# unclearness/vacancy

Hardware: AMD Instinct MI355X
Metric: Mvoxel*views/s (Carve) (higher is better)
Workload: dtype f32

## Files before the change

### vacancy_amd/csrc/carve_fused_device.h

```cpp
#pragma once
#include "carve_fused.h"

namespace vcy {
namespace {

#define VCY_SETPRIO(n) __builtin_amdgcn_s_setprio(n)

#ifdef VCY_PHASE_TIMING
__device__ unsigned long long g_phase_ticks[256][16];
#define VCY_PT_DECL unsigned long long pt_last = __builtin_amdgcn_s_memtime(), pt_acc[16] = {0, 0, 0, 0, 0, 0, 0, 0, 0, 0, 0, 0, 0, 0, 0, 0}
#define VCY_PT(slot)                                                  \
  do {                                                                \
    const unsigned long long t_ = __builtin_amdgcn_s_memtime();       \
    pt_acc[slot] += t_ - pt_last;                                     \
    pt_last = t_;                                                     \
  } while (0)
#define VCY_PT_COUNT(slot) pt_acc[slot] += 1
#define VCY_PT_FLUSH(lane_)                                                                         \
  do {                                                                                              \
    if ((lane_) == 0)                                                                               \
      for (int q_ = 0; q_ < 16; ++q_) atomicAdd(&g_phase_ticks[blockIdx.x & 255][q_], pt_acc[q_]);  \
  } while (0)
#else
#define VCY_PT_DECL
// ... 27 lines not shown
}

__device__ __forceinline__ float div_view1(int div, float n, float d) {
  float r = __builtin_amdgcn_rcpf(d);
  if (div == 1) {
    const float e = __builtin_fmaf(-d, r, 1.0f);
    r = __builtin_fmaf(e, r, r);
  }
  const float q = n * r;
  const float e2 = __builtin_fmaf(-d, q, n);
  return __builtin_fmaf(e2, r, q);
}

__device__ __forceinline__ bool in_fast_div_range(float z) {
  const unsigned lo = 0x21800000u;
  const unsigned hi = 0x5d800000u;
  return (__float_as_uint(z) - lo) <= (hi - lo);
}

typedef const float __attribute__((address_space(1))) * gfloat_ptr;
__device__ __forceinline__ float load_u32_index(gfloat_ptr base, unsigned idx) {
  typedef const char __attribute__((address_space(1))) * gchar_ptr;
  return *(gfloat_ptr)((gchar_ptr)base + (idx << 2));
}
typedef const float __attribute__((address_space(4))) * cfloat_ptr;
__device__ __attribute__((noinline)) bool sample_generic(const ViewParams* v, ModeParams m, float px,
                                                         float py, float pz, float* dist) {
  return view_distance<true, 0, 0, false, false>(*v, m, px, py, pz, dist);
}

__device__ __forceinline__ void wave_lds_fence() {
  __builtin_amdgcn_fence(__ATOMIC_RELEASE, "wavefront");
  __builtin_amdgcn_wave_barrier();
  __builtin_amdgcn_fence(__ATOMIC_ACQUIRE, "wavefront");
}

__device__ __forceinline__ float rcp_count(float m) {
  const float r = __builtin_amdgcn_rcpf(m);
  const float e = __builtin_fmaf(-m, r, 1.0f);
  return __builtin_fmaf(e, r, r);
}

template <int UPDATE>
__device__ __forceinline__ bool apply_sample(bool ok, float dist, float wgt, float& s, int& n) {
  if (UPDATE == VCY_UPDATE_MAX) {
    const bool take = ok && (n < 1 || dist > s);
    s = take ? dist : s;
    n += take ? 1 : 0;
    return take;
  } else if (UPDATE == kUpdateWaUnitWeight) {
    const float inv_denom = rcp_count((float)(n + 1));
    const float avg = ((float)n * s + dist) * inv_denom;
    const float ns = (n < 1) ? dist : avg;
    s = ok ? ns : s;
    n += ok ? 1 : 0;
  } else {
    const float inv_denom = div_fast(1.0f, wgt * (float)(n + 1));
    const float avg = (wgt * (float)n * s + wgt * dist) * inv_denom;
    const float ns = (n < 1) ? dist : avg;
    s = ok ? ns : s;
    n += ok ? 1 : 0;
  }
  return ok;
}

__device__ __forceinline__ void update_max_touched(float dist, float& s, int& n, unsigned long long& took) {
  asm("v_cmp_gt_f32_e32 vcc, %[d], %[s]\n\t"
      "s_or_b64 %[took], %[took], vcc\n\t"
      "v_cndmask_b32_e32 %[s], %[s], %[d], vcc\n\t"
      "v_addc_co_u32_e32 %[n], vcc, 0, %[n], vcc"
      : [s] "+v"(s), [n] "+v"(n), [took] "+s"(took)
      : [d] "v"(dist)
      : "vcc");
}

template <bool TRUNC>
__device__ __forceinline__ void update_wa_unit(float dist, float& s, float& fn, unsigned long long& took) {
  const float f1 = fn + 1.0f;
  const float avg = (fn * s + dist) * rcp_count(f1);
  if (TRUNC) {
    asm("v_cmp_ngt_f32_e32 vcc, -1.0, %[d]\n\t"
        "s_or_b64 %[took], %[took], vcc\n\t"
        "v_cndmask_b32_e32 %[s], %[s], %[avg], vcc\n\t"
        "v_cndmask_b32_e32 %[fn], %[fn], %[f1], vcc"
        : [s] "+v"(s), [fn] "+v"(fn), [took] "+s"(took)
        : [d] "v"(dist), [avg] "v"(avg), [f1] "v"(f1)
        : "vcc");
  } else {
    s = avg;
    fn = f1;
  }
}

typedef float f4 __attribute__((ext_vector_type(4)));
typedef f4 __attribute__((address_space(3))) lds_float4;

template <int UPDATE>
__device__ __forceinline__ bool apply_sample(bool ok, float dist, float wgt, float& s, float& fn) {
  const float f1 = fn + 1.0f;
  float avg;
  if (UPDATE == kUpdateWaUnitWeight) {
    avg = (fn * s + dist) * rcp_count(f1);
  } else {
    avg = (wgt * fn * s + wgt * dist) * div_fast(1.0f, wgt * f1);
  }
  const float ns = (fn < 1.0f) ? dist : avg;
  s = ok ? ns : s;
  fn = ok ? f1 : fn;
  return ok;
}

__device__ __forceinline__ int div_small(int q, float inv) { return (int)(((float)q + 0.5f) * inv); }

typedef float __attribute__((address_space(3))) lds_float;
typedef uint32_t __attribute__((address_space(3))) lds_u32;

__device__ __forceinline__ void raw_prefetch(const ViewParams& v, const TileInfo& ti, int lane, float* buf) {
#ifdef VCY_FLOOR_NO_TILE_LOADS
  return;
#endif
  asm volatile("" : "+v"(lane));
  const int nq = __builtin_amdgcn_readfirstlane(ti.nq);
  if (nq == 0) return;
  const int th = __builtin_amdgcn_readfirstlane(ti.th);
  const int tx0 = __builtin_amdgcn_readfirstlane(ti.tx0);
  const int ty0 = __builtin_amdgcn_readfirstlane(ti.ty0);
  gfloat_ptr img = (gfloat_ptr)v.sdf;
  const unsigned width = (unsigned)v.width;
  lds_float* dst = (lds_float*)buf;
  if (tx0 + 15 <= v.roi_max_xi && ty0 + 15 <= v.roi_max_yi) {
    const unsigned lane_off = __umul24(width, (unsigned)lane >> 4) + ((unsigned)lane & 15u);
    gfloat_ptr base = img + (__umul24(width, (unsigned)ty0) + (unsigned)tx0);
#pragma unroll
    for (int r = 0; r < 4; ++r) {
      if (4 * r <= th)
        __builtin_amdgcn_global_load_lds(base + (size_t)(4 * r) * width + lane_off, dst + 64 * r, 4, 0, 0);
    }
    return;
  }
  const unsigned xx = (unsigned)min(tx0 + (lane & 15), v.roi_max_xi);
  const int yl = ty0 + (lane >> 4);
#pragma unroll
  for (int r = 0; r < 4; ++r) {
    if (4 * r <= th) {
      const unsigned yy = (unsigned)min(yl + 4 * r, v.roi_max_yi);
      __builtin_amdgcn_global_load_lds(img + (__umul24(width, yy) + xx), dst + 64 * r, 4, 0, 0);
    }
  }
}

__device__ __forceinline__ void raw_tile_wait() { asm volatile("s_waitcnt vmcnt(0)" ::: "memory"); }

__device__ __forceinline__ float wave_min(float v) {
#define VCY_DPP_MIN(CTRL) asm volatile("s_nop 1\n\tv_min_f32_dpp %0, %0, %0 " CTRL : "+v"(v))
  VCY_DPP_MIN("quad_perm:[1,0,3,2] row_mask:0xf bank_mask:0xf");
  VCY_DPP_MIN("quad_perm:[2,3,0,1] row_mask:0xf bank_mask:0xf");
  VCY_DPP_MIN("row_half_mirror row_mask:0xf bank_mask:0xf");
  VCY_DPP_MIN("row_mirror row_mask:0xf bank_mask:0xf");
  VCY_DPP_MIN("row_bcast:15 row_mask:0xa bank_mask:0xf");
  VCY_DPP_MIN("row_bcast:31 row_mask:0xc bank_mask:0xf");
#undef VCY_DPP_MIN
  return __uint_as_float(__builtin_amdgcn_readlane(__float_as_uint(v), 63));
}

__device__ __forceinline__ void tile_fill(const ViewParams& v, const TileInfo& ti, int lane, float* tile) {
  const int nq = __builtin_amdgcn_readfirstlane(ti.nq);
  if (nq == 0) return;
  const int tw = __builtin_amdgcn_readfirstlane(ti.tw), th = __builtin_amdgcn_readfirstlane(ti.th);
  const int tx0 = __builtin_amdgcn_readfirstlane(ti.tx0);
  const int ty0 = __builtin_amdgcn_readfirstlane(ti.ty0);
  const float inv_pitch = __uint_as_float(__builtin_amdgcn_readfirstlane(__float_as_uint(ti.inv_tw)));
  const int pitch = tw + 1, npx = pitch * (th + 1);
  gfloat_ptr img = (gfloat_ptr)v.sdf;
  const unsigned width = (unsigned)v.width;
  lds_float* dst = (lds_float*)tile;
  for (int q0 = 0; q0 < npx; q0 += 64) {
    const int q = q0 + lane;
    if (q < npx) {
      const int j = div_small(q, inv_pitch), i = q - j * pitch;
      const unsigned xx = (unsigned)min(tx0 + i, v.roi_max_xi), yy = (unsigned)min(ty0 + j, v.roi_max_yi);
      __builtin_amdgcn_global_load_lds(img + (__umul24(width, yy) + xx), dst + q0, 4, 0, 0);
    }
  }
  raw_tile_wait();
}

template <bool SAMEF, int TQ, bool GEN>
__device__ __forceinline__ TileInfo footprint_of(const FusedView& fv, float xl, float xh, float yl, float yh, float zl_,
                                                 float zh, bool is_ortho, bool outside_max, bool want_bound,
                                                 bool want_lower, float* lower_out = nullptr) {
  const ViewParams& v = fv.v;
  const float xa = fmaxf(fabsf(xl), fabsf(xh)), ya = fmaxf(fabsf(yl), fabsf(yh)), za = fmaxf(fabsf(zl_), fabsf(zh));
  const bool ortho = GEN && is_ortho;
  float p0[3], ax[3], ay[3], az[3], mag[3];
#pragma unroll
  for (int i = 0; i < 3; ++i) {
    p0[i] = v.t[i] + (v.r[i][0] * xl + (v.r[i][1] * yl + v.r[i][2] * zl_));
    ax[i] = v.r[i][0] * (xh - xl);
    ay[i] = v.r[i][1] * (yh - yl);
    az[i] = v.r[i][2] * (zh - zl_);
    mag[i] = fabsf(v.t[i]) + (fabsf(v.r[i][0]) * xa + (fabsf(v.r[i][1]) * ya + fabsf(v.r[i][2]) * za));
  }
  float umin = INFINITY, umax = -INFINITY, wmin = INFINITY, wmax_ = -INFINITY, zmin = INFINITY, zmax = -INFINITY;
  int bad = 0;
  const float fx = v.fx, fy = SAMEF ? v.fx : v.fy;
  float pxy[4][3];
#pragma unroll
  for (int i = 0; i < 3; ++i) {
    pxy[0][i] = p0[i];
    pxy[1][i] = p0[i] + ax[i];
    pxy[2][i] = p0[i] + ay[i];
    pxy[3][i] = pxy[1][i] + ay[i];
  }
#pragma unroll
  for (int corner = 0; corner < 8; ++corner) {
    float pc[3];
#pragma unroll
    for (int i = 0; i < 3; ++i) pc[i] = (corner & 4) ? pxy[corner & 3][i] + az[i] : pxy[corner & 3][i];
    float u = pc[0], w = pc[1];
    if (!ortho) {
      const float rz = __builtin_amdgcn_rcpf(pc[2]);
      u = __builtin_fmaf(fx * rz, pc[0], v.cx);
      w = __builtin_fmaf(fy * rz, pc[1], v.cy);
    }
    umin = fminf(umin, u);
    umax = fmaxf(umax, u);
    wmin = fminf(wmin, w);
    wmax_ = fmaxf(wmax_, w);
    zmin = fminf(zmin, pc[2]);
    zmax = fmaxf(zmax, pc[2]);
  }
  if (!ortho) bad |= !in_fast_div_range(zmin) || !in_fast_div_range(zmax);
  bad |= !(mag[0] < 0x1p60f) || !(mag[1] < 0x1p60f) || !(mag[2] < 0x1p60f);
  bad |= !(umin > -1.0e6f) || !(umax < 1.0e6f) || !(wmin > -1.0e6f) || !(wmax_ < 1.0e6f);
  const float uabs = fmaxf(fabsf(umin), fabsf(umax)), wabs = fmaxf(fabsf(wmin), fabsf(wmax_));
  float err_u, err_w;
  if (ortho) {
    err_u = 0x1p-21f * mag[0];
    err_w = 0x1p-21f * mag[1];
  } else {
    bad |= !(zmin * 4.0f >= zmax);
    const float iz = 0x1p-21f * __builtin_amdgcn_rcpf(zmin) * 1.0001f;
    err_u = iz * (fx * mag[0] + (uabs + fabsf(v.cx)) * mag[2]) + 0x1p-21f * (uabs + fabsf(v.cx));
    err_w = iz * (fy * mag[1] + (wabs + fabsf(v.cy)) * mag[2]) + 0x1p-21f * (wabs + fabsf(v.cy));
  }
  const float margin = 0.125f;
  bad |= !(err_u <= 0.03125f) || !(err_w <= 0.03125f);
  TileInfo ti;
  ti.lo_x = ti.lo_y = INFINITY;
  ti.hi_x = ti.hi_y = -INFINITY;
  ti.pitchf = 0.0f;
  ti.base = 0;
  ti.tx0 = ti.ty0 = ti.tw = ti.nq = ti.th = 0;
  ti.inv_tw = 1.0f;
  ti.ub = INFINITY;
  ti.sure = 0;
  if (!bad) {
    const int tx0 = max((int)floorf(umin - margin), v.roi_min_xi);
    const int ty0 = max((int)floorf(wmin - margin), v.roi_min_yi);
    const int tx1 = min((int)floorf(umax + margin), v.roi_max_xi);
    const int ty1 = min((int)floorf(wmax_ + margin), v.roi_max_yi);
    const int tw = tx1 - tx0 + 1, th = ty1 - ty0 + 1;
    constexpr bool kRaw = TQ == kTileRaw;
    if (tw > 0 && th > 0 && (kRaw ? (tw <= 15 && th <= 15) : ((tw + 1) * (th + 1) <= kBigPixels))) {
      const bool unclipped = (int)floorf(umin - margin) >= v.roi_min_xi && (int)floorf(wmin - margin) >= v.roi_min_yi &&
                             (int)floorf(umax + margin) < v.roi_max_xi && (int)floorf(wmax_ + margin) < v.roi_max_yi;
      const bool depth_ok = 0x1p-20f * mag[2] <= 0.25f * zmin && zmin >= 0x1p-58f && zmax <= 0x1p58f;
      const int pitch = kRaw ? 16 : tw + 1;
      const bool small_base = ty0 * pitch + tx0 < (1 << 18);
      const bool depth_ok_ortho = zmin > 0x1p-20f * mag[2];
      ti.sure = (unclipped && (ortho ? depth_ok_ortho : depth_ok) && small_base) ? 1 : 0;
      ti.tx0 = tx0;
      ti.ty0 = ty0;
      ti.tw = tw;
      ti.th = th;
      ti.nq = tw * th;
      ti.inv_tw = 1.0f / (float)pitch;
      ti.pitchf = (float)pitch;
      ti.base = -(ty0 * pitch + tx0);
      ti.lo_x = (float)tx0;
      ti.lo_y = (float)ty0;
      ti.hi_x = (tx1 == v.roi_max_xi) ? v.roi_max_x
                                      : __uint_as_float(__float_as_uint((float)(tx1 + 1)) - 1u);
      ti.hi_y = (ty1 == v.roi_max_yi) ? v.roi_max_y
                                      : __uint_as_float(__float_as_uint((float)(ty1 + 1)) - 1u);
      if (want_bound) {
        const int pw = min(tx1 + 1, v.roi_max_xi) - tx0 + 1;
        const int ph = min(ty1 + 1, v.roi_max_yi) - ty0 + 1;
        float m = -INFINITY;
        int has_nan = 0;
        gfloat_ptr wm = (gfloat_ptr)fv.wmax;
        const int L = min(pw, ph) >= 8 ? 3 : 2;
        const int k = 1 << L;
        const int nxw = (pw + k - 1) >> L, nyw = (ph + k - 1) >> L;
        const bool small = nxw <= 3 && nyw <= 3;
        const int ux = __any(small && nxw >= 3) ? 3 : (__any(small && nxw >= 2) ? 2 : 1);
        const int uy = __any(small && nyw >= 3) ? 3 : (__any(small && nyw >= 2) ? 2 : 1);
        if (wm != nullptr) {
          gfloat_ptr lvl = wm + (L == 3 ? (size_t)fv.wmax_plane : (size_t)0);
          const unsigned origin = __umul24((unsigned)v.width, (unsigned)ty0) + (unsigned)tx0 + (L == 3 ? (unsigned)fv.wmax_plane : 0u);
          if (nxw <= 3 && nyw <= 3) {
            float t[9];
#pragma unroll
            for (int bq = 0; bq < 3; ++bq) {
              const unsigned ro = origin + __umul24((unsigned)v.width, (unsigned)min(bq << L, max(ph - k, 0)));
#pragma unroll
              for (int aq = 0; aq < 3; ++aq) {
                t[3 * bq + aq] = -INFINITY;
                if (aq < ux && bq < uy) t[3 * bq + aq] = load_u32_index(wm, ro + (unsigned)min(aq << L, max(pw - k, 0)));
              }
            }
#pragma unroll
            for (int q = 0; q < 9; ++q) m = fmaxf(m, t[q]);
// ... 90 lines not shown
```

### vacancy_amd/csrc/carve_fused_kernel.h

```cpp
#pragma once
#include <cstdio>
#include <cstdlib>
#include <type_traits>

#include "carve_fused_device.h"

namespace vcy {
namespace {

template <int UPDATE, bool CHECKMAX, int TQ, bool GEN, int NB>
constexpr int carve_waves_per_simd() {
  if (NB > 1) return NB > 2 ? 4 : 5;
  if (GEN || CHECKMAX || TQ != kTileRaw || UPDATE == VCY_UPDATE_WEIGHTED_AVERAGE) return VCY_WAVES_CHECKED;
  if (UPDATE == kUpdateWaUnitWeight) return NB == 0 ? VCY_WAVES_WA_ONE : VCY_WAVES_WA;
  return NB == 0 ? VCY_WAVES_ONE : VCY_WAVES;
}
template <typename CountT, int UPDATE, bool TRUNC, bool SAMEF, bool CHECKMAX, int TQ, bool GEN, int DIV, int NB = 1>
__global__ __launch_bounds__(64 * (NB > 1 ? kRowWaves : kWgWaves))
__attribute__((amdgpu_waves_per_eu(NB > 1 ? 1 : carve_waves_per_simd<UPDATE, CHECKMAX, TQ, GEN, NB>(),
                                   carve_waves_per_simd<UPDATE, CHECKMAX, TQ, GEN, NB>()))) void carve_fused_kernel(GridParams g,
                                                          const FusedView* __restrict__ views,
                                                          const float* __restrict__ c0_all,
                                                          int nviews_arg, ModeParams mode, int nbx,
                                                          int nby, BlockDecode bd, int cull_enabled, int state_flags,
// ... 291 lines not shown
  } else if (vec_io) {
    float4 a, b4;
    CountVec cv;
    if (kOne && eager) {
      a = make_float4(eager_a.x, eager_a.y, eager_a.z, eager_a.w), b4 = make_float4(eager_b.x, eager_b.y, eager_b.z, eager_b.w);
      cv = eager_c;
    } else {
      a = *(const float4*)(g.sdf + row0 + x_first), b4 = *(const float4*)(g.sdf + row0 + x_first + 4);
      cv = *(const CountVec*)(cnt + row0 + x_first);
    }
    prefetch_first_tile();
    s[0] = a.x, s[1] = a.y, s[2] = a.z, s[3] = a.w, s[4] = b4.x, s[5] = b4.y, s[6] = b4.z, s[7] = b4.w;
#pragma unroll
    for (int k = 0; k < WX; ++k) n[k] = (NT)cv[k];
  } else {
#pragma unroll
    for (int k = 0; k < WX; ++k) {
      const int xk = min(x_first + k, g.nx - 1);
      s[k] = g.sdf[row0 + xk];
      n[k] = (NT)cnt[row0 + xk];
    }
  }

  bool all_touched = false;
  auto refresh_all_touched = [&]() {
    if (UPDATE != VCY_UPDATE_MAX || all_touched) return;
    NT nmin = n[0];
#pragma unroll
    for (int k = 1; k < WX; ++k) nmin = min(nmin, n[k]);
    all_touched = __all(nmin >= (NT)1);
  };
  if (!fresh && !kRows) refresh_all_touched();
  bool none_touched = fresh != 0;
  auto refresh_none_touched = [&]() {
    NT nmax = n[0];
#pragma unroll
    for (int k = 1; k < WX; ++k) nmax = max(nmax, n[k]);
    none_touched = __all(nmax < (NT)1);
  };
  if (!kRows && !fresh && UPDATE == VCY_UPDATE_MAX && !all_touched) refresh_none_touched();
  bool uniform_cnt = false;
  float fnu = 0.0f;
  auto refresh_uniform_cnt = [&]() {
    if (UPDATE == VCY_UPDATE_MAX) return;
    if (fresh) {
      uniform_cnt = true;
      fnu = 0.0f;
    } else {
      const float f0 = __uint_as_float(__builtin_amdgcn_readfirstlane(__float_as_uint((float)n[0])));
      bool same = true;
#pragma unroll
      for (int k = 0; k < WX; ++k) same = same && (float)n[k] == f0;
      uniform_cnt = __all(same);
      fnu = f0;
    }
  };
  if (!kRows) refresh_uniform_cnt();
  auto leave_uniform = [&]() {
    if (!uniform_cnt) return;
    uniform_cnt = false;
#pragma unroll
    for (int k = 0; k < WX; ++k) n[k] = (NT)fnu;
  };
  int jc = -1;
  auto live_views = [&]() -> unsigned long long {
    bool drop = false;
    if (want_bound) {
      if (TRUNC) drop = ub_lane < -1.0f;
      if (UPDATE == VCY_UPDATE_MAX && all_touched) {
        float m = s[0];
#pragma unroll
        for (int k = 1; k < WX; ++k) m = fminf(m, s[k]);
        const float smin = wave_min(m);
        drop = drop || ub_lane <= smin;
      }
    }
    if constexpr (kRows) {
      const unsigned long long cur_bits = 0xffull << (8 * jc);
      return (live & ~cur_bits) | (__ballot(!drop) & view_mask & cur_bits);
    }
    return __ballot(!drop) & view_mask;
  };
  const int vi_end = kRows ? 64 : nviews;
  auto next_view = [&](unsigned long long live, int after) -> int {
    const unsigned long long rest = (after >= 63) ? 0ull : (live & ~((2ull << after) - 1ull));
    return rest ? (__ffsll((long long)rest) - 1) : vi_end;
  };

  unsigned long long changed_lanes = 0ull;
  if (!kRows) live = live_views();
  int vi = live ? (__ffsll((long long)live) - 1) : vi_end;
  if (kRaw && vi < vi_end && vi != vi_pre) raw_prefetch(views[kRows ? (vi & 7) : vi].v, tile_of(vi), lane, raw_buf(0));
  typedef CountT CountVecR __attribute__((ext_vector_type(WX)));
  typedef CountVecR __attribute__((address_space(3))) lds_countvec_r;
  auto finish_brick = [&]() {
    if constexpr (kRows) {
      leave_uniform();
      if (brick_min != nullptr && implied) {
        float m = s[0];
#pragma unroll
        for (int k = 1; k < WX; ++k) m = fminf(m, s[k]);
        const float smin = wave_min(m);
        if (lane == 0) brick_min[brick_lin] = smin;
      }
      lds_float4* rs = (lds_float4*)(float4*)(stage_s + (jc * 64 + lane) * WX);
      rs[0] = f4{s[0], s[1], s[2], s[3]};
      rs[1] = f4{s[4], s[5], s[6], s[7]};
      CountVecR cv;
#pragma unroll
      for (int k = 0; k < WX; ++k) cv[k] = (CountT)n[k];
      *(lds_countvec_r*)(CountVecR*)(stage_n + (jc * 64 + lane) * WX) = cv;
      if (lane == 0) stage_mask[jc] = fresh ? ~0ull : changed_lanes;
    }
  };
  auto begin_brick = [&](int j) {
    if constexpr (kRows) {
      jc = j;
      x_first = x_seg + j * WX;
      brick_lin = brick_seg + j;
      changed_lanes = 0ull;
      if (fresh) {
#pragma unroll
        for (int k = 0; k < WX; ++k) {
          s[k] = kInvalidSdf;
          n[k] = (NT)0;
        }
      } else {
        const lds_float4* rs = (const lds_float4*)(float4*)(stage_s + (j * 64 + lane) * WX);
        const f4 a = rs[0], b4 = rs[1];
        const CountVecR cv = *(const lds_countvec_r*)(CountVecR*)(stage_n + (j * 64 + lane) * WX);
        s[0] = a.x, s[1] = a.y, s[2] = a.z, s[3] = a.w, s[4] = b4.x, s[5] = b4.y, s[6] = b4.z, s[7] = b4.w;
#pragma unroll
        for (int k = 0; k < WX; ++k) n[k] = (NT)cv[k];
      }
      all_touched = false;
      none_touched = fresh != 0;
      if (!fresh) {
        refresh_all_touched();
        if (UPDATE == VCY_UPDATE_MAX && !all_touched) refresh_none_touched();
      }
      refresh_uniform_cnt();
    }
  };
  VCY_PT(0);
  VCY_PT_COUNT(10);

#if defined(VCY_DEV_EXIT_AT) && VCY_DEV_EXIT_AT == 4
  {
    coop_leave();
    return;
  }
#endif
  int n_processed = 0;
  while (vi < vi_end) {
    if constexpr (kRows) {
      if ((vi >> 3) != jc) {
        raw_tile_wait();
        wave_lds_fence();
        if (jc >= 0) finish_brick();
        begin_brick(vi >> 3);
        live = live_views();
        if (((live >> vi) & 1ull) == 0ull) {
          vi = next_view(live, vi);
          if (vi < vi_end) raw_prefetch(views[vi & 7].v, tile_of(vi), lane, raw_buf(cur));
          continue;
        }
      }
    }
    const int vv = kRows ? (vi & 7) : vi;
    const ViewParams& v = views[vv].v;
    cfloat_ptr c0 = (cfloat_ptr)(c0_all + ((size_t)vv * (nxp / WX) + (x_first / WX)) * kC0Stride);
    VCY_SETPRIO(3);
    wave_lds_fence();
    if (kRaw) {
      raw_tile_wait();
    } else {
      tile_fill(v, tile_of(vi), lane, (float*)tile);
    }
    wave_lds_fence();
    int vnext = next_view(live, vi);
    if (kRaw && vnext < vi_end) raw_prefetch(views[kRows ? (vnext & 7) : vnext].v, tile_of(vnext), lane, raw_buf(cur ^ 1));
    ++n_processed;
    const float pitchf = tile_of(vi).pitchf;
    const int base = tile_of(vi).base;
    const int big_pitch = kRaw ? 16 : (int)pitchf;
    const lds_float* rawcur = (const lds_float*)raw_buf(cur);
    auto quad_at = [&](unsigned idx) -> float4 {
      if constexpr (kRaw) {
        const lds_float* p = rawcur + idx;
        return make_float4(p[0], p[1], p[16], p[17]);
      } else {
        const lds_float* p = (const lds_float*)(float*)tile + idx;
        const lds_float* p2 = p + big_pitch;
        return make_float4(p[0], p[1], p2[0], p2[1]);
      }
    };

    const float lo_x = tile_of(vi).lo_x, hi_x = tile_of(vi).hi_x;
    const float lo_y = tile_of(vi).lo_y, hi_y = tile_of(vi).hi_y;
    const bool is_ortho = GEN && mode.ortho != 0, is_nn = GEN && mode.interp == VCY_INTERP_NN;
    const float h12x = v.r[0][1] * py + v.r[0][2] * pz, h12y = v.r[1][1] * py + v.r[1][2] * pz;
    const float h12z = v.r[2][1] * py + v.r[2][2] * pz;
    VCY_SETPRIO(0);
    VCY_PT(1);

    auto carve_view = [&](auto sure_tag) {
      constexpr bool SURE = decltype(sure_tag)::value;
      bool slow[WX];
      bool any_slow = false;
      bool moved = false;
#pragma unroll
      for (int k = 0; k < WX; ++k) {
        const float pcz = v.t[2] + (c0[16 + k] + h12z);
        float qx = 1.0f, qy = 1.0f;
        if (!is_ortho) {
          qx = div_view<DIV>(v.fx, pcz);
          qy = SAMEF ? qx : div_view<DIV>(v.fy, pcz);
        }
        const float pcx = v.t[0] + (c0[2 * k] + h12x), pcy = v.t[1] + (c0[2 * k + 1] + h12y);
        const float u = is_ortho ? pcx : qx * pcx + v.cx;
        const float w = is_ortho ? pcy : qy * pcy + v.cy;
        bool in_tile = true;
        if (!SURE) {
          const bool zfast = is_ortho ? !(pcz < 0.0f) : in_fast_div_range(pcz);
          in_tile = zfast && u >= lo_x && u <= hi_x && w >= lo_y && w <= hi_y;
          slow[k] = !in_tile;
          any_slow = any_slow || !in_tile;
        }
        const float fu = floorf(u), fw = floorf(w);
        const float lu = u - fu, lv = w - fw;
        const float mu = 1.0f - lu, mv = 1.0f - lv;
        unsigned idx = (unsigned)((int)__builtin_fmaf(fw, pitchf, fu) + base);
        if (!SURE) idx = min(idx, (unsigned)(kRaw ? 256 - 18 : max(kBigPixels - big_pitch - 2, 0)));
        const float4 q = quad_at(idx);
        float dist = ((((mu * mv) * q.x) + ((lu * mv) * q.y)) + ((mu * lv) * q.z)) + ((lu * lv) * q.w);
        if (is_nn) {
          const float top = lu >= 0.5f ? q.y : q.x, bot = lu >= 0.5f ? q.w : q.z;
          dist = lv >= 0.5f ? bot : top;
        }
        bool ok = in_tile;
        if (TRUNC) ok = ok && !(dist < -1.0f);
        if (CHECKMAX) ok = ok && !(n[k] > (NT)g.max_update_num);
        moved = apply_sample<UPDATE>(ok, dist, g.weight, s[k], n[k]) || moved;
      }
      if (!SURE && any_slow) {
#pragma unroll
        for (int k = 0; k < WX; ++k) {
          if (slow[k]) {
            float dist = 0.0f;
            bool ok = sample_generic(&v, mode, g.px[min(x_first + k, g.nx - 1)], py, pz, &dist);
            if (CHECKMAX) ok = ok && !(n[k] > (NT)g.max_update_num);
            moved = apply_sample<UPDATE>(ok, dist, g.weight, s[k], n[k]) || moved;
          }
        }
      }
      const unsigned long long mv = __ballot(moved);
      changed_lanes |= mv;
      return mv != 0ull;
    };
    constexpr bool kFastMax = UPDATE == VCY_UPDATE_MAX && !TRUNC && !CHECKMAX;
    constexpr bool kFastWa = UPDATE == kUpdateWaUnitWeight && !CHECKMAX;
    constexpr bool kFastWaGeneral = UPDATE == VCY_UPDATE_WEIGHTED_AVERAGE && !CHECKMAX;
    auto carve_view_fast = [&](auto first_tag, auto notrunc_tag, auto uniform_tag) -> bool {
      constexpr bool FIRST = decltype(first_tag)::value;
      constexpr bool NOTRUNC = decltype(notrunc_tag)::value;
      constexpr bool UNIFORM = decltype(uniform_tag)::value;
      float fn_v = 0.0f, inv_v = 0.0f, wgt_v = 1.0f;
      if constexpr (UNIFORM) {
        const float f1 = fnu + 1.0f;
        asm volatile("v_mov_b32_e32 %0, %1" : "=v"(fn_v) : "s"(fnu));
        if constexpr (UPDATE == kUpdateWaUnitWeight) {
          inv_v = rcp_count(fn_v + 1.0f);
        } else {
          asm volatile("v_mov_b32_e32 %0, %1" : "=v"(wgt_v) : "s"(g.weight));
          inv_v = div_fast(1.0f, wgt_v * (fn_v + 1.0f));
          fn_v = wgt_v * fn_v;
        }
        fnu = f1;
      }
      float pitch16, cmagic;
      constexpr int kElemB = 4;
      constexpr float kAddrUnit = 0x1p-149f;
      {
        const float p16 = pitchf * ((float)kElemB * kAddrUnit);
        const unsigned lds_off = kRaw ? (unsigned)(size_t)rawcur : (unsigned)(size_t)(const lds_float*)(float*)tile;
        const int ci = kElemB * base + (int)lds_off;
        const float cm = ci < 0 ? -__int_as_float(-ci) : __int_as_float(ci);
        asm volatile("v_mov_b32_e32 %0, %1" : "=v"(pitch16) : "s"(p16));
        asm volatile("v_mov_b32_e32 %0, %1" : "=v"(cmagic) : "s"(cm));
      }
      unsigned long long took = 0;
      constexpr int kGroup = VCY_FAST_GROUP;
#pragma unroll
      for (int k0 = 0; k0 < WX; k0 += kGroup) {
        float lu[kGroup], lv[kGroup];
        f4 q[kGroup];
#pragma unroll
        for (int j = 0; j < kGroup; ++j) {
          const int k = k0 + j;
          const float pcz = v.t[2] + (c0[16 + k] + h12z);
          const float qx = div_view<DIV>(v.fx, pcz);
          const float qy = SAMEF ? qx : div_view<DIV>(v.fy, pcz);
          const float pcx = v.t[0] + (c0[2 * k] + h12x), pcy = v.t[1] + (c0[2 * k + 1] + h12y);
          float u = qx * pcx + v.cx, w = qy * pcy + v.cy;
          if constexpr (GEN) {
            if (is_ortho) u = pcx, w = pcy;
          }
          const float fu = floorf(u), fw = floorf(w);
          lu[j] = u - fu;
          lv[j] = w - fw;
          const float a = __builtin_fmaf(fw, pitch16, __builtin_fmaf(fu, (float)kElemB * kAddrUnit, cmagic));
          const unsigned addr = __float_as_uint(a);
          const lds_float* tp = (const lds_float*)(size_t)addr;
          if constexpr (kRaw) {
            q[j] = f4{tp[0], tp[1], tp[16], tp[17]};
          } else {
            const lds_float* tp2 = tp + big_pitch;
            q[j] = f4{tp[0], tp[1], tp2[0], tp2[1]};
          }
        }
#pragma unroll
        for (int j = 0; j < kGroup; ++j) {
          const int k = k0 + j;
          const float mu = 1.0f - lu[j], mv = 1.0f - lv[j];
          float dist =
              ((((mu * mv) * q[j].x) + ((lu[j] * mv) * q[j].y)) + ((mu * lv[j]) * q[j].z)) + ((lu[j] * lv[j]) * q[j].w);
          if constexpr (GEN) {
            if (is_nn) {
              const float top = lu[j] >= 0.5f ? q[j].y : q[j].x, bot = lu[j] >= 0.5f ? q[j].w : q[j].z;
              dist = lv[j] >= 0.5f ? bot : top;
            }
          }
          if constexpr (FIRST) {
            s[k] = dist;
            n[k] = (NT)1;
          } else if constexpr (kFastMax) {
            update_max_touched(dist, s[k], n[k], took);
          } else if constexpr (UNIFORM) {
            if constexpr (UPDATE == kUpdateWaUnitWeight) s[k] = (fn_v * s[k] + dist) * inv_v;
            else s[k] = (fn_v * s[k] + wgt_v * dist) * inv_v;
          } else if constexpr (kFastWa) {
            update_wa_unit<TRUNC && !NOTRUNC>(dist, s[k], n[k], took);
          }
        }
      }
      constexpr bool kConditional = !FIRST && !UNIFORM && (kFastMax || (kFastWa && TRUNC && !NOTRUNC));
      changed_lanes |= kConditional ? took : ~0ull;
      return (kFastMax && !FIRST) ? took != 0ull : true;
    };
    bool brick_moved;
    const int sure_bits = __builtin_amdgcn_readfirstlane(tile_of(vi).sure);
    const bool sure = (sure_bits & 1) != 0, never_truncated = (sure_bits & 2) != 0;
    constexpr bool kHasFast = kFastMax || kFastWa || kFastWaGeneral;
    const bool fast_first = kFastMax && sure && none_touched;
    const bool fast_next = (kFastMax && sure && all_touched) || (kFastWa && sure && implied);
    const bool fast_general = kFastWaGeneral && sure && uniform_cnt && (!TRUNC || never_truncated);
    if (kFastWaGeneral && __builtin_expect_with_probability(fast_general, 1, 0.9)) {
      if (fnu < 1.0f) {
        brick_moved = carve_view_fast(std::true_type{}, std::false_type{}, std::false_type{});
        fnu = 1.0f;
      } else {
        brick_moved = carve_view_fast(std::false_type{}, std::true_type{}, std::true_type{});
      }
      VCY_PT(2);
      VCY_PT_COUNT(7);
    } else if (__builtin_expect_with_probability(fast_next, kHasFast && !kFastWaGeneral, 0.9)) {
      const bool all_updated = kFastWa && (!TRUNC || never_truncated);
      if (kFastWa && all_updated && uniform_cnt) {
        brick_moved = carve_view_fast(std::false_type{}, std::true_type{}, std::true_type{});
      } else if (kFastWa && all_updated) {
        brick_moved = carve_view_fast(std::false_type{}, std::true_type{}, std::false_type{});
      } else {
        if (kFastWa) leave_uniform();
        brick_moved = carve_view_fast(std::false_type{}, std::false_type{}, std::false_type{});
      }
      VCY_PT(2);
      VCY_PT_COUNT(7);
    } else if (__builtin_expect_with_probability(fast_first, kHasFast, 0.99)) {
      brick_moved = carve_view_fast(std::true_type{}, std::false_type{}, std::false_type{});
      VCY_PT(2);
      VCY_PT_COUNT(7);
    } else if (sure) {
      leave_uniform();
      brick_moved = carve_view(std::true_type{});
      VCY_PT(3);
      VCY_PT_COUNT(8);
    } else {
      leave_uniform();
      brick_moved = carve_view(std::false_type{});
      VCY_PT(4);
      VCY_PT_COUNT(9);
    }
    VCY_SETPRIO(3);
    if (brick_moved) VCY_PT_COUNT(11);
    none_touched = false;
    if (!kOne) refresh_all_touched();

    if (!kOne && want_bound && UPDATE == VCY_UPDATE_MAX && brick_moved) {
      live = live_views();
      const int v2 = next_view(live, vi);
      if (v2 != vnext) {
        vnext = v2;
        if (kRaw && vnext < vi_end) raw_prefetch(views[kRows ? (vnext & 7) : vnext].v, tile_of(vnext), lane, raw_buf(cur ^ 1));
      }
    }
    vi = vnext;
    cur ^= 1;
    VCY_PT(5);
  }

  if constexpr (kRows) {
    if (jc >= 0) finish_brick();
    wave_lds_fence();
    if (pair_count != nullptr && lane == 0) atomicAdd(&pair_count[bz], (unsigned long long)n_processed);
    {
      const int yw = by * BY + (lane >> 3), c16 = lane & 7, jw = c16 >> 1;
      const unsigned long long mw = jw < NB ? stage_mask[jw] : 0ull;
      const bool col_ok = jw < NB && yw < g.ny && x_seg + 4 * c16 < g.nx;
#pragma unroll
      for (int i = 0; i < BZ; ++i) {
        const int row = 8 * i + (lane >> 3);
        if (zl0 + i < g.nz_local && col_ok && ((mw >> row) & 1ull) != 0ull) {
          const f4 q = *(const lds_float4*)(float4*)(stage_s + (jw * 64 + row) * WX + (c16 & 1) * 4);
          *(float4*)(g.sdf + (((int64_t)(zl0 + i) * g.ny + yw) * g.nx + x_seg + 4 * c16)) = make_float4(q.x, q.y, q.z, q.w);
        }
      }
      const int jn = lane & 3;
      const unsigned long long mn = jn < NB ? stage_mask[jn] : 0ull;
#pragma unroll
      for (int i = 0; i < 4; ++i) {
        const int row = 16 * i + (lane >> 2);
        const int yn = by * BY + (row & 7), zn = zl0 + (row >> 3);
        if (jn < NB && yn < g.ny && zn < g.nz_local && x_seg + WX * jn < g.nx && ((mn >> row) & 1ull) != 0ull) {
          const CountVecR cv = *(const lds_countvec_r*)(CountVecR*)(stage_n + (jn * 64 + row) * WX);
          *(CountVecR*)(cnt + (((int64_t)zn * g.ny + yn) * g.nx + x_seg + WX * jn)) = cv;
        }
      }
    }
    return;
  }
  leave_uniform();
  int tid_w = (int)threadIdx.x;
  asm volatile("" : "+v"(tid_w));
  const int lane_w = tid_w & 63;
  const int y_w = by * BY + (lane_w & (BY - 1)), zl_w = zl0 + (lane_w >> 3);
  const bool lane_valid_w = y_w < g.ny && zl_w < g.nz_local;
  const int64_t row0_w = ((int64_t)min(zl_w, g.nz_local - 1) * g.ny + min(y_w, g.ny - 1)) * g.nx;
#if defined(VCY_DEV_EXIT_AT) && VCY_DEV_EXIT_AT == 5
  {
    coop_leave();
    return;
  }
#endif
  if (pair_count != nullptr && lane == 0) atomicAdd(&pair_count[bz], (unsigned long long)n_processed);
  if (brick_min != nullptr && implied) {
    float m = s[0];
#pragma unroll
    for (int k = 1; k < WX; ++k) m = fminf(m, s[k]);
    const float smin = wave_min(m);
    if (lane == 0) brick_min[brick_lin] = smin;
  }
  if (coop) {
    const bool changed = lane_valid_w && (fresh != 0 || ((changed_lanes >> lane_w) & 1ull) != 0ull);
    const unsigned long long my_mask = __ballot(changed);
    {
      lds_float4* rs = (lds_float4*)(float4*)(coop_s + lane_w * kCoopSdfPitch + wave * WX);
      rs[0] = f4{s[0], s[1], s[2], s[3]};
      rs[1] = f4{s[4], s[5], s[6], s[7]};
      CountVec8 cv;
#pragma unroll
      for (int k = 0; k < WX; ++k) cv[k] = (CountT)n[k];
      *(lds_countvec*)(CountVec8*)(coop_n + lane_w * coop_cnt_pitch<CountT>() + wave * WX) = cv;
      if (lane == 0) coop_mask[wave] = my_mask, coop_mask[kWgWaves + wave] = 1ull;
    }
    __syncthreads();
    int n_here = 0, my_rank = 0;
#pragma unroll
    for (int w = 0; w < kWgWaves; ++w) {
      const int here = __builtin_amdgcn_readfirstlane((int)coop_mask[kWgWaves + w]);
      n_here += here;
      my_rank += (w < wave) ? here : 0;
    }
    const int xb = bx * BX;
    constexpr int kSdfChunks = 2 * kWgWaves, kSdfRows = 64 / kSdfChunks;
    for (int gi = my_rank; gi < 64 / kSdfRows; gi += n_here) {
      const int r = gi * kSdfRows + lane / kSdfChunks, ch = lane % kSdfChunks;
      if ((coop_mask[ch >> 1] >> r) & 1ull) {
        const f4 v = *(lds_float4*)(float4*)(coop_s + r * kCoopSdfPitch + ch * 4);
        const int64_t rowg = ((int64_t)(zl0 + (r >> 3)) * g.ny + (by * BY + (r & 7))) * g.nx;
        if (nt_store) __builtin_nontemporal_store(v, (f4*)(g.sdf + rowg + xb + ch * 4));
        else *(float4*)(g.sdf + rowg + xb + ch * 4) = make_float4(v.x, v.y, v.z, v.w);
      }
    }
    constexpr int kCntRows = 64 / kWgWaves;
    for (int gi = my_rank; gi < 64 / kCntRows; gi += n_here) {
      const int r = gi * kCntRows + lane / kWgWaves, ch = lane % kWgWaves;
      if ((coop_mask[ch] >> r) & 1ull) {
        const CountVec8 cv = *(lds_countvec*)(CountVec8*)(coop_n + r * coop_cnt_pitch<CountT>() + ch * WX);
        const int64_t rowg = ((int64_t)(zl0 + (r >> 3)) * g.ny + (by * BY + (r & 7))) * g.nx;
        if (nt_store) __builtin_nontemporal_store(cv, (CountVec8*)(cnt + rowg + xb + ch * WX));
        else *(CountVec8*)(cnt + rowg + xb + ch * WX) = cv;
      }
    }
  } else if (lane_valid_w) {
    if (vec_io) {
      bool changed = fresh != 0;
#ifdef VCY_FLOOR_NO_STORES
      {
        float ssum = 0.0f, nsum = 0.0f;
#pragma unroll
        for (int k = 0; k < WX; ++k) ssum += s[k], nsum += (float)n[k];
        changed = ssum == 1.2345e-30f && nsum == 777.25f;
      }
#else
      changed = changed || ((changed_lanes >> lane_w) & 1ull) != 0ull;
#endif
      if (changed) {
        *(float4*)(g.sdf + row0_w + x_first) = make_float4(s[0], s[1], s[2], s[3]);
        *(float4*)(g.sdf + row0_w + x_first + 4) = make_float4(s[4], s[5], s[6], s[7]);
        CountVec cv;
#pragma unroll
        for (int k = 0; k < WX; ++k) cv[k] = (CountT)n[k];
        *(CountVec*)(cnt + row0_w + x_first) = cv;
      }
    } else {
#pragma unroll
      for (int k = 0; k < WX; ++k) {
        if (x_first + k < g.nx) {
          const int64_t idx = row0_w + x_first + k;
          if (fresh || ((changed_lanes >> lane_w) & 1ull) != 0ull) {
            g.sdf[idx] = s[k];
            cnt[idx] = (CountT)n[k];
          }
        }
      }
    }
  }
  VCY_PT(6);
  VCY_PT_FLUSH(lane);
}

template <typename CountT, int UPDATE, bool TRUNC, bool SAMEF, bool CHECKMAX, int TQ, bool GEN, int DIV, int NB>
void launch_instance(const CarveLaunch& l) {
  constexpr bool kRows = NB > 1;
  const size_t coop = (l.state_flags & kStateCoopStore) ? coop_lds_bytes<CountT>() : 0;
  const size_t lds = kRows    ? (size_t)kRowWaves * row_lds_bytes_per_wave<CountT, NB>()
                     : NB == 0 ? (size_t)kWgWaves * 64 * sizeof(float4) + coop
                               : (size_t)kWgWaves * tile_f4_per_wave<TQ>() * sizeof(float4) +
                                     (size_t)kWgWaves * l.n_views * sizeof(TileInfo) + coop;
  const BlockDecode bd = make_block_decode(kRows ? (unsigned)l.row_units : l.grid_x, l.nbx, l.nby);
  hipLaunchKernelGGL((carve_fused_kernel<CountT, UPDATE, TRUNC, SAMEF, CHECKMAX, TQ, GEN, DIV, NB>), dim3(l.grid_x),
                     dim3(64 * (kRows ? kRowWaves : kWgWaves)), lds, l.stream, l.g, l.views, l.c0_all,
                     NB == 0 ? 1 : l.n_views, l.mode, l.nbx, l.nby, bd, l.cull, l.state_flags, l.records, l.nbricks,
                     l.brick_min, l.wg_list, l.pair_count);
}

template <int... Vs, typename F>
void with_constant(int value, F&& f) {
  if (!((value == Vs && (f(std::integral_constant<int, Vs>{}), true)) || ...)) {
    fprintf(stderr, "carve_fused_kernel: no instance for selection %d\n", value);
    abort();
// ... 48 lines not shown
```

Before: 4.373 million.

## Add tight inner loop for consecutive fast max-update views; merge DPP min asm

Refactors per-view setup and teardown into begin_view/end_view lambdas and, for the max-update fast path, loops directly over successive 'sure' views without going back through the outer dispatch and brick checks. View parameters are reached through a constant-address-space pointer so loads can be scalar. The wave_min DPP sequence is folded into one asm block so the compiler cannot schedule between the steps. The aim is lower per-view control overhead. The cost is more code and register pressure from the duplicated template instantiation, and the loop exits must keep brick boundaries and the all_touched state correct.

```diff
diff --git a/vacancy_amd/csrc/carve_fused_device.h b/vacancy_amd/csrc/carve_fused_device.h
--- a/vacancy_amd/csrc/carve_fused_device.h
+++ b/vacancy_amd/csrc/carve_fused_device.h
@@ -203,13 +203,14 @@
 __device__ __forceinline__ void raw_tile_wait() { asm volatile("s_waitcnt vmcnt(0)" ::: "memory"); }
 
 __device__ __forceinline__ float wave_min(float v) {
-#define VCY_DPP_MIN(CTRL) asm volatile("s_nop 1\n\tv_min_f32_dpp %0, %0, %0 " CTRL : "+v"(v))
-  VCY_DPP_MIN("quad_perm:[1,0,3,2] row_mask:0xf bank_mask:0xf");
-  VCY_DPP_MIN("quad_perm:[2,3,0,1] row_mask:0xf bank_mask:0xf");
-  VCY_DPP_MIN("row_half_mirror row_mask:0xf bank_mask:0xf");
-  VCY_DPP_MIN("row_mirror row_mask:0xf bank_mask:0xf");
-  VCY_DPP_MIN("row_bcast:15 row_mask:0xa bank_mask:0xf");
-  VCY_DPP_MIN("row_bcast:31 row_mask:0xc bank_mask:0xf");
+#define VCY_DPP_MIN(CTRL) "s_nop 1\n\tv_min_f32_dpp %0, %0, %0 " CTRL "\n\t"
+  asm volatile(VCY_DPP_MIN("quad_perm:[1,0,3,2] row_mask:0xf bank_mask:0xf")
+               VCY_DPP_MIN("quad_perm:[2,3,0,1] row_mask:0xf bank_mask:0xf")
+               VCY_DPP_MIN("row_half_mirror row_mask:0xf bank_mask:0xf")
+               VCY_DPP_MIN("row_mirror row_mask:0xf bank_mask:0xf")
+               VCY_DPP_MIN("row_bcast:15 row_mask:0xa bank_mask:0xf")
+               VCY_DPP_MIN("row_bcast:31 row_mask:0xc bank_mask:0xf")
+               : "+v"(v));
 #undef VCY_DPP_MIN
   return __uint_as_float(__builtin_amdgcn_readlane(__float_as_uint(v), 63));
 }
diff --git a/vacancy_amd/csrc/carve_fused_kernel.h b/vacancy_amd/csrc/carve_fused_kernel.h
--- a/vacancy_amd/csrc/carve_fused_kernel.h
+++ b/vacancy_amd/csrc/carve_fused_kernel.h
@@ -467,6 +467,64 @@
   }
 #endif
   int n_processed = 0;
+  const bool is_ortho = GEN && mode.ortho != 0, is_nn = GEN && mode.interp == VCY_INTERP_NN;
+  typedef const ViewParams __attribute__((address_space(4))) cview;
+  cview* vp = nullptr;
+  cfloat_ptr c0 = nullptr;
+  int vnext = vi_end;
+  float pitchf = 0.0f;
+  int base = 0, big_pitch = 0;
+  const lds_float* rawcur = nullptr;
+  float h12x = 0.0f, h12y = 0.0f, h12z = 0.0f;
+  auto begin_view = [&]() {
+    const int vv = kRows ? (vi & 7) : vi;
+    const ViewParams& v = views[vv].v;
+    vp = (cview*)&v;
+    c0 = (cfloat_ptr)(c0_all + ((size_t)vv * (nxp / WX) + (x_first / WX)) * kC0Stride);
+    VCY_SETPRIO(3);
+    wave_lds_fence();
+    if (kRaw) {
+      raw_tile_wait();
+    } else {
+      tile_fill(v, tile_of(vi), lane, (float*)tile);
+    }
+    wave_lds_fence();
+    vnext = next_view(live, vi);
+    if (kRaw && vnext < vi_end) raw_prefetch(views[kRows ? (vnext & 7) : vnext].v, tile_of(vnext), lane, raw_buf(cur ^ 1));
+    ++n_processed;
+    pitchf = tile_of(vi).pitchf;
+    base = tile_of(vi).base;
+    big_pitch = kRaw ? 16 : (int)pitchf;
+    rawcur = (const lds_float*)raw_buf(cur);
+    h12x = vp->r[0][1] * py + vp->r[0][2] * pz, h12y = vp->r[1][1] * py + vp->r[1][2] * pz;
+    h12z = vp->r[2][1] * py + vp->r[2][2] * pz;
+    VCY_SETPRIO(0);
+    VCY_PT(1);
+  };
+  auto end_view = [&](bool brick_moved) {
+    VCY_SETPRIO(3);
+    if (brick_moved) VCY_PT_COUNT(11);
+    none_touched = false;
+    if (!kOne) refresh_all_touched();
+
+    if (!kOne && want_bound && UPDATE == VCY_UPDATE_MAX && brick_moved) {
+      live = live_views();
+      const int v2 = next_view(live, vi);
+      if (v2 != vnext) {
+        vnext = v2;
+        if (kRaw && vnext < vi_end) raw_prefetch(views[kRows ? (vnext & 7) : vnext].v, tile_of(vnext), lane, raw_buf(cur ^ 1));
+      }
+    }
+    vi = vnext;
+    cur ^= 1;
+    VCY_PT(5);
+  };
+  auto next_fast_bits = [&]() -> int {
+    if (kOne || vi >= vi_end) return 0;
+    if (kRows && (vi >> 3) != jc) return 0;
+    const int bits = __builtin_amdgcn_readfirstlane(tile_of(vi).sure);
+    return (bits & 1) != 0 ? bits : 0;
+  };
   while (vi < vi_end) {
     if constexpr (kRows) {
       if ((vi >> 3) != jc) {
@@ -482,24 +540,7 @@
         }
       }
     }
-    const int vv = kRows ? (vi & 7) : vi;
-    const ViewParams& v = views[vv].v;
-    cfloat_ptr c0 = (cfloat_ptr)(c0_all + ((size_t)vv * (nxp / WX) + (x_first / WX)) * kC0Stride);
-    VCY_SETPRIO(3);
-    wave_lds_fence();
-    if (kRaw) {
-      raw_tile_wait();
-    } else {
-      tile_fill(v, tile_of(vi), lane, (float*)tile);
-    }
-    wave_lds_fence();
-    int vnext = next_view(live, vi);
-    if (kRaw && vnext < vi_end) raw_prefetch(views[kRows ? (vnext & 7) : vnext].v, tile_of(vnext), lane, raw_buf(cur ^ 1));
-    ++n_processed;
-    const float pitchf = tile_of(vi).pitchf;
-    const int base = tile_of(vi).base;
-    const int big_pitch = kRaw ? 16 : (int)pitchf;
-    const lds_float* rawcur = (const lds_float*)raw_buf(cur);
+    begin_view();
     auto quad_at = [&](unsigned idx) -> float4 {
       if constexpr (kRaw) {
         const lds_float* p = rawcur + idx;
@@ -511,16 +552,11 @@
       }
     };
 
-    const float lo_x = tile_of(vi).lo_x, hi_x = tile_of(vi).hi_x;
-    const float lo_y = tile_of(vi).lo_y, hi_y = tile_of(vi).hi_y;
-    const bool is_ortho = GEN && mode.ortho != 0, is_nn = GEN && mode.interp == VCY_INTERP_NN;
-    const float h12x = v.r[0][1] * py + v.r[0][2] * pz, h12y = v.r[1][1] * py + v.r[1][2] * pz;
-    const float h12z = v.r[2][1] * py + v.r[2][2] * pz;
-    VCY_SETPRIO(0);
-    VCY_PT(1);
-
     auto carve_view = [&](auto sure_tag) {
       constexpr bool SURE = decltype(sure_tag)::value;
+      cview& v = *vp;
+      const float lo_x = tile_of(vi).lo_x, hi_x = tile_of(vi).hi_x;
+      const float lo_y = tile_of(vi).lo_y, hi_y = tile_of(vi).hi_y;
       bool slow[WX];
       bool any_slow = false;
       bool moved = false;
@@ -563,7 +599,7 @@
         for (int k = 0; k < WX; ++k) {
           if (slow[k]) {
             float dist = 0.0f;
-            bool ok = sample_generic(&v, mode, g.px[min(x_first + k, g.nx - 1)], py, pz, &dist);
+            bool ok = sample_generic((const ViewParams*)vp, mode, g.px[min(x_first + k, g.nx - 1)], py, pz, &dist);
             if (CHECKMAX) ok = ok && !(n[k] > (NT)g.max_update_num);
             moved = apply_sample<UPDATE>(ok, dist, g.weight, s[k], n[k]) || moved;
           }
@@ -580,6 +616,7 @@
       constexpr bool FIRST = decltype(first_tag)::value;
       constexpr bool NOTRUNC = decltype(notrunc_tag)::value;
       constexpr bool UNIFORM = decltype(uniform_tag)::value;
+      cview& v = *vp;
       float fn_v = 0.0f, inv_v = 0.0f, wgt_v = 1.0f;
       if constexpr (UNIFORM) {
         const float f1 = fnu + 1.0f;
@@ -666,7 +703,6 @@
     bool brick_moved;
     const int sure_bits = __builtin_amdgcn_readfirstlane(tile_of(vi).sure);
     const bool sure = (sure_bits & 1) != 0, never_truncated = (sure_bits & 2) != 0;
-    constexpr bool kHasFast = kFastMax || kFastWa || kFastWaGeneral;
     const bool fast_first = kFastMax && sure && none_touched;
     const bool fast_next = (kFastMax && sure && all_touched) || (kFastWa && sure && implied);
     const bool fast_general = kFastWaGeneral && sure && uniform_cnt && (!TRUNC || never_truncated);
@@ -679,7 +715,21 @@
       }
       VCY_PT(2);
       VCY_PT_COUNT(7);
-    } else if (__builtin_expect_with_probability(fast_next, kHasFast && !kFastWaGeneral, 0.9)) {
+    } else if (kFastMax && __builtin_expect_with_probability(fast_next || fast_first, 1, 0.99)) {
+      auto run = [&](auto first_tag) -> bool {
+        brick_moved = carve_view_fast(first_tag, std::false_type{}, std::false_type{});
+        VCY_PT(2);
+        VCY_PT_COUNT(7);
+        end_view(brick_moved);
+        if (!all_touched || (next_fast_bits() & 1) == 0) return false;
+        begin_view();
+        return true;
+      };
+      bool more = true;
+      if (fast_first) more = run(std::true_type{});
+      while (more) more = run(std::false_type{});
+      continue;
+    } else if (kFastWa && __builtin_expect_with_probability(fast_next, 1, 0.9)) {
       const bool all_updated = kFastWa && (!TRUNC || never_truncated);
       if (kFastWa && all_updated && uniform_cnt) {
         brick_moved = carve_view_fast(std::false_type{}, std::true_type{}, std::true_type{});
@@ -689,10 +739,6 @@
         if (kFastWa) leave_uniform();
         brick_moved = carve_view_fast(std::false_type{}, std::false_type{}, std::false_type{});
       }
-      VCY_PT(2);
-      VCY_PT_COUNT(7);
-    } else if (__builtin_expect_with_probability(fast_first, kHasFast, 0.99)) {
-      brick_moved = carve_view_fast(std::true_type{}, std::false_type{}, std::false_type{});
       VCY_PT(2);
       VCY_PT_COUNT(7);
     } else if (sure) {
@@ -706,22 +752,7 @@
       VCY_PT(4);
       VCY_PT_COUNT(9);
     }
-    VCY_SETPRIO(3);
-    if (brick_moved) VCY_PT_COUNT(11);
-    none_touched = false;
-    if (!kOne) refresh_all_touched();
-
-    if (!kOne && want_bound && UPDATE == VCY_UPDATE_MAX && brick_moved) {
-      live = live_views();
-      const int v2 = next_view(live, vi);
-      if (v2 != vnext) {
-        vnext = v2;
-        if (kRaw && vnext < vi_end) raw_prefetch(views[kRows ? (vnext & 7) : vnext].v, tile_of(vnext), lane, raw_buf(cur ^ 1));
-      }
-    }
-    vi = vnext;
-    cur ^= 1;
-    VCY_PT(5);
+    end_view(brick_moved);
   }
 
   if constexpr (kRows) {
```

New measurement: 4.557 million, median of 6. 1.04x the previous value.
